# maxsonate/video-diffusion-nnx

Measured on AMD Instinct MI355X. Metric: denoised frames/sec, 16fx64x64 1000-step DDPM, higher is better.
Workload: dtype bf16; 1 GPU; config_v2_2 (north-star shape): Unet3D dim=64 C=1, 16f x 64x64, DDPM T=1000 p_sample_loop (UNet forward + p_sample per step, hipGraph replay); value = n_gpus*B*F/(T*s_per_step); batch_per_gpu=64, parallelism=dp1 (independent samples, no collective), mfma_operands=bf16, storage=weights fp32 master, activations bf16, fp32 accumulate, process_group=none (single process)

## Files before the change

### video_diffusion_nnx_amd/csrc/conv_igemm.hip

```cpp
#include "vdx_common.h"
#include <type_traits>
#include "vdx_internal.h"
#include "vdx_glds.h"
#include "model.h"
#include <stdlib.h>
#include <string.h>

namespace vdx {

typedef unsigned u32x4 __attribute__((ext_vector_type(4)));
typedef unsigned u32x2 __attribute__((ext_vector_type(2)));
constexpr unsigned OOB = 0xFFFFFFF0u;

template <int MODE, int BC, int TN, int NW, int INF>
__global__ __launch_bounds__(64 * NW, (NW == 8 && TN == 2) ? 4 : 2) void conv_igemm_kernel(const ConvArgs P) {
    using M = Mma<MODE>;
    constexpr int KT = M::KT;
    constexpr int RS = ROW_STRIDE;
    constexpr int WAVES_C = BC / 64;
    constexpr int WAVES_P = NW / WAVES_C;
    constexpr int NT = 64 * NW;
    constexpr int TM = 4;
    constexpr int APIECES = KT / 4;
    constexpr int WREGS = BC * 8 / NT;
// ... 732 lines not shown
    const int lp = lane & 15, q = lane >> 4;
    const int tiles_x = P.W >> 4, tiles_pf = tiles_x * (P.H >> 4);
    const int t0 = blockIdx.x * tiles_per_block, t1 = min(t0 + tiles_per_block, total_tiles);
    if (t0 >= t1) return;

    uint4 wf[9][2][2];
#pragma unroll
    for (int tap = 0; tap < 9; ++tap)
#pragma unroll
        for (int ch = 0; ch < 2; ++ch)
#pragma unroll
            for (int tm = 0; tm < 2; ++tm)
                wf[tap][ch][tm] = *reinterpret_cast<const uint4*>(reinterpret_cast<const char*>(P.wp) +
                    ((size_t)tap * P.wrows + P.wrow0 + wc * 32 + 8 * (lp >> 2) + 4 * tm + (lp & 3)) * 128 + ch * 64 + q * 16);
    if (tid < 128) chs[tid] = 0.0;
    if (tid < 64) biasl[tid] = P.bias ? P.bias[tid] : 0.f;

    const char* const zero_page = reinterpret_cast<const char*>(g_zero_page_c64d);
    const char* const xb = reinterpret_cast<const char*>(P.x0);
    const unsigned al_base = lds_addr(Al);
    auto decode = [&](int t, int& f, int& ty, int& tx) { f = t / tiles_pf; const int r = t - f * tiles_pf; ty = r / tiles_x; tx = r - ty * tiles_x; };
    auto dma = [&](int t, int buf) {
        int f, ty, tx; decode(t, f, ty, tx);
        int ln = lane;
        asm volatile("" : "+v"(ln));
        const unsigned dst = al_base + buf * C64D_APL + wave_u * 1024;
#pragma unroll
        for (int k = 0; k < NK; ++k) {
            if (wave_u + 8 * k >= NDMA) continue;
            const int hp = (wave_u + 8 * k) * 8 + (ln >> 3);
            const int hy = (hp * 3641) >> 16, hx = hp - hy * 18;
            const int gy = ty * 16 - 1 + hy, gx = tx * 16 - 1 + hx;
            const bool ok = hp < C64_HALO && gy >= 0 && gy < P.H && gx >= 0 && gx < P.W;
            const size_t off = (size_t)((f * P.H + gy) * P.W + gx) * 128 + (((ln & 7) ^ (hx & 7)) << 4);
            glds16(ok ? static_cast<const void*>(xb + off) : static_cast<const void*>(zero_page), dst + k * 8 * 1024);
        }
    };
    const __amdgpu_buffer_rsrc_t rsy = __builtin_amdgcn_make_buffer_rsrc(P.y, 0, (unsigned)P.NF * P.H * P.W * 64u * (OUT16 ? 2u : 4u), 0x00020000);
    f32x4 ssum[2], ssq[2];
#pragma unroll
    for (int i = 0; i < 2; ++i) { ssum[i] = f32x4{0.f, 0.f, 0.f, 0.f}; ssq[i] = f32x4{0.f, 0.f, 0.f, 0.f}; }
    auto flush_stats = [&](int b) {
        if (!P.out_stats) return;
#pragma unroll
        for (int tm = 0; tm < 2; ++tm)
#pragma unroll
            for (int e = 0; e < 4; ++e) {
                const float s1 = reduce16(ssum[tm][e]), s2 = reduce16(ssq[tm][e]);
                const int c = wc * 32 + 8 * q + 4 * tm + e;
                if (lp == 0) { unsafeAtomicAdd(&chs[c], (double)s1); unsafeAtomicAdd(&chs[64 + c], (double)s2); }
                ssum[tm][e] = 0.f; ssq[tm][e] = 0.f;
            }
        __syncthreads();
        const int cpg = 64 / P.out_groups;
        int tt = tid;
        asm volatile("" : "+v"(tt));
        if (tt < 2 * P.out_groups) {
            const int g = tt >> 1, which = tt & 1;
            double t = 0.0;
            for (int c = g * cpg; c < (g + 1) * cpg; ++c) t += chs[which * 64 + c];
            unsafeAtomicAdd(P.out_stats + (((size_t)b * GN_SLOTS + (blockIdx.x % GN_SLOTS)) * P.out_groups + g) * 2 + which, t);
        }
        __syncthreads();
        if (tid < 128) chs[tid] = 0.0;
        __syncthreads();
    };

    int bdx[3][2];
#pragma unroll
    for (int ch = 0; ch < 2; ++ch)
#pragma unroll
        for (int dx = 0; dx < 3; ++dx) { const int hx = lp + dx; bdx[dx][ch] = hx * 128 + 16 * ((q + 4 * ch) ^ (hx & 7)); }
    const int rowbase = (4 * wp) * 18 * 128;

    int fcur, tyc, txc;
    decode(t0, fcur, tyc, txc);
    int bcur = fcur / P.F;
    __syncthreads();
    dma(t0, 0);
    if (t0 + 1 < t1) { dma(t0 + 1, 1); wait_vm<5>(); } else wait_vm<0>();
    __syncthreads();
    int buf = 0;
    for (int t = t0; t < t1; ++t) {
        const bool more = t + 1 < t1, more2 = t + 2 < t1;
        int fn = fcur, tyn = tyc, txn = txc, bn = bcur;
        if (more) { decode(t + 1, fn, tyn, txn); bn = fn / P.F; }
        if (more2) dma(t + 2, buf >= 1 ? buf - 1 : 2);
        const char* At = Al + buf * C64D_APL + rowbase;
        const int oy0 = tyc * 16 + 4 * wp, ox = txc * 16 + lp;
        f32x4 acc[2][4];
        uint4 bf[2][3];
        auto frag_read = [&](uint4 (&d)[3], int hr, int ch) {
#pragma unroll
            for (int dx = 0; dx < 3; ++dx) d[dx] = *reinterpret_cast<const uint4*>(At + bdx[dx][ch] + hr * (18 * 128));
        };
        frag_read(bf[0], 0, 0);
#pragma unroll
        for (int hr = 0; hr < 6; ++hr) {
            if (hr < 4) { acc[0][hr] = f32x4{0.f, 0.f, 0.f, 0.f}; acc[1][hr] = f32x4{0.f, 0.f, 0.f, 0.f}; }
#pragma unroll
            for (int ch = 0; ch < 2; ++ch) {
                const int s_ = 2 * hr + ch;
                if (s_ + 1 < 12) frag_read(bf[(s_ + 1) & 1], (s_ + 1) >> 1, (s_ + 1) & 1);
                __builtin_amdgcn_sched_barrier(0);
#pragma unroll
                for (int dx = 0; dx < 3; ++dx)
#pragma unroll
                    for (int dy = 0; dy < 3; ++dy) {
                        const int tn = hr - dy;
                        if (tn < 0 || tn > 3) continue;
#pragma unroll
                        for (int tm = 0; tm < 2; ++tm) M::mma(acc[tm][tn], wf[dy * 3 + dx][ch][tm], bf[s_ & 1][dx]);
                    }
                __builtin_amdgcn_sched_barrier(0);
            }
            if (hr >= 2) {
                const int tn = hr - 2;
                float4 bias4[2];
#pragma unroll
                for (int tm = 0; tm < 2; ++tm) bias4[tm] = *reinterpret_cast<const float4*>(biasl + wc * 32 + 8 * q + 4 * tm);
                const unsigned gout = (unsigned)(((fcur * P.H + oy0 + tn) * P.W + ox) * 64 + wc * 32 + 8 * q);
                float4 v[2];
#pragma unroll
                for (int tm = 0; tm < 2; ++tm) {
                    v[tm] = make_float4(acc[tm][tn][0] + bias4[tm].x, acc[tm][tn][1] + bias4[tm].y, acc[tm][tn][2] + bias4[tm].z, acc[tm][tn][3] + bias4[tm].w);
                    ssum[tm][0] += v[tm].x; ssum[tm][1] += v[tm].y; ssum[tm][2] += v[tm].z; ssum[tm][3] += v[tm].w;
                    ssq[tm][0] += v[tm].x * v[tm].x; ssq[tm][1] += v[tm].y * v[tm].y; ssq[tm][2] += v[tm].z * v[tm].z; ssq[tm][3] += v[tm].w * v[tm].w;
                }
                if constexpr (OUT16)
                    __builtin_amdgcn_raw_buffer_store_b128(u32x4{pack_bf16x2(v[0].x, v[0].y), pack_bf16x2(v[0].z, v[0].w), pack_bf16x2(v[1].x, v[1].y), pack_bf16x2(v[1].z, v[1].w)}, rsy, gout * 2u, 0, 0);
                else {
#pragma unroll
                    for (int tm = 0; tm < 2; ++tm)
                        __builtin_amdgcn_raw_buffer_store_b128(u32x4{__float_as_uint(v[tm].x), __float_as_uint(v[tm].y), __float_as_uint(v[tm].z), __float_as_uint(v[tm].w)}, rsy, (gout + 4 * tm) * 4u, 0, 0);
                }
            }
        }
        constexpr int NST = OUT16 ? 4 : 8;
        if (more2) wait_vm<5 + NST>(); else wait_vm<NST>();
        if (more && bn != bcur) { flush_stats(bcur); bcur = bn; }
        fcur = fn; tyc = tyn; txc = txn;
        buf = buf == 2 ? 0 : buf + 1;
        __syncthreads();
    }
    flush_stats(bcur);
}

#ifndef VDX_C64Q_VPM
#define VDX_C64Q_VPM 6
#endif
template <int CIN, bool PRO, bool OUT16, int COUT = 64>
__global__ __launch_bounds__(512) void conv64q_kernel(const ConvArgs P, const int tiles_per_block, const int total_tiles) {
    using M = Mma<MODE_BF16>;
    static_assert(CIN == 64 || (CIN == 128 && !PRO), "prologue form: 64 input channels");
    static_assert(COUT == 64 || (COUT == 32 && !PRO), "COUT");
    constexpr int NWC = COUT / 16, NWP = 8 / NWC, RW = 16 / NWP, NHR = RW + 2, NSTEP = 2 * NHR;
    constexpr int NPL = CIN / 64;
    constexpr int NDMA = 41, NK = (NDMA + 7) / 8;
    constexpr int NST = (OUT16 ? 1 : 2) * (RW / 2);
    extern __shared__ __attribute__((aligned(16))) char smem[];
    char* Al = smem;
    double* chs = reinterpret_cast<double*>(Al + 3 * C64D_APL);
    float* biasl = reinterpret_cast<float*>(chs + 128);
    float* coefA = biasl + 64;
    float* coefD = coefA + 64;
    float* gmean = coefD + 64;

    const int tid = threadIdx.x, lane = tid & 63;
    const int wave_u = __builtin_amdgcn_readfirstlane(tid >> 6);
    const int wc = wave_u % NWC, wp = wave_u / NWC;
    const int lp = lane & 15, q = lane >> 4;
    const int tiles_x = P.W >> 4, tiles_pf = tiles_x * (P.H >> 4);
    const int t0 = blockIdx.x * tiles_per_block, t1 = min(t0 + tiles_per_block, total_tiles);
    if (t0 >= t1) return;

    uint4 wf[9][CIN / 32];
#pragma unroll
    for (int tap = 0; tap < 9; ++tap)
#pragma unroll
        for (int c = 0; c < CIN / 32; ++c)
            wf[tap][c] = *reinterpret_cast<const uint4*>(reinterpret_cast<const char*>(P.wp) +
                ((size_t)tap * P.wrows + P.wrow0 + wc * 16 + lp) * (CIN * 2) + c * 64 + q * 16);
    if (tid < 128) chs[tid] = 0.0;
    if (tid < 64) biasl[tid] = (P.bias && tid < COUT) ? P.bias[tid] : 0.f;

    const char* const zero_page = reinterpret_cast<const char*>(g_zero_page_c64d);
    const char* const xb0 = reinterpret_cast<const char*>(P.x0);
    const char* const xb1 = (CIN == 128) ? (P.C1 ? reinterpret_cast<const char*>(P.x1) : xb0 + 128) : xb0;
    const int rowb = (CIN == 128 && !P.C1) ? 256 : 128;
    const bool split32 = CIN == 64 && P.C1 == 32;
    const char* const xs1 = split32 ? reinterpret_cast<const char*>(P.x1) : nullptr;
    const unsigned al_base = lds_addr(Al);
    auto decode = [&](int t, int& f, int& ty, int& tx) { f = t / tiles_pf; const int r = t - f * tiles_pf; ty = r / tiles_x; tx = r - ty * tiles_x; };
    auto dma = [&](int t, int plane, int buf) {
        int f, ty, tx; decode(t, f, ty, tx);
        int ln = lane;
        asm volatile("" : "+v"(ln));
        const char* const xb = plane ? xb1 : xb0;
        const unsigned dst = al_base + buf * C64D_APL + wave_u * 1024;
#pragma unroll
        for (int k = 0; k < NK; ++k) {
            if (wave_u + 8 * k >= NDMA) continue;
            const int hp = (wave_u + 8 * k) * 8 + (ln >> 3);
            const int hy = (hp * 3641) >> 16, hx = hp - hy * 18;
            const int gy = ty * 16 - 1 + hy, gx = tx * 16 - 1 + hx;
            const bool ok = hp < C64_HALO && gy >= 0 && gy < P.H && gx >= 0 && gx < P.W;
            const int cch = (ln & 7) ^ (hx & 7);
            const size_t pixi = (size_t)((f * P.H + gy) * P.W + gx);
            const char* src = split32 ? (cch < 4 ? xb0 : xs1) + pixi * 64 + ((cch & 3) << 4) : xb + pixi * rowb + (cch << 4);
            glds16(ok ? static_cast<const void*>(src) : static_cast<const void*>(zero_page), dst + k * 8 * 1024);
        }
    };
    const __amdgpu_buffer_rsrc_t rsy = __builtin_amdgcn_make_buffer_rsrc(P.y, 0, (unsigned)P.NF * P.H * P.W * (unsigned)COUT * (OUT16 ? 2u : 4u), 0x00020000);
    float ssum[8], ssq[8];
#pragma unroll
    for (int i = 0; i < 8; ++i) { ssum[i] = 0.f; ssq[i] = 0.f; }
    auto flush_stats = [&](int b) {
        if (!P.out_stats) return;
#pragma unroll
        for (int i = 0; i < 8; ++i) {
            const float s1 = reduce16(ssum[i]), s2 = reduce16(ssq[i]);
            const int c = wc * 16 + 8 * (q >> 1) + i;
            if (lp == 0) { unsafeAtomicAdd(&chs[c], (double)s1); unsafeAtomicAdd(&chs[64 + c], (double)s2); }
            ssum[i] = 0.f; ssq[i] = 0.f;
        }
        __syncthreads();
        const int cpg = COUT / P.out_groups;
        int tt = tid;
        asm volatile("" : "+v"(tt));
        if (tt < 2 * P.out_groups) {
            const int g = tt >> 1, which = tt & 1;
            double t = 0.0;
            for (int c = g * cpg; c < (g + 1) * cpg; ++c) t += chs[which * 64 + c];
            unsafeAtomicAdd(P.out_stats + (((size_t)b * GN_SLOTS + (blockIdx.x % GN_SLOTS)) * P.out_groups + g) * 2 + which, t);
        }
        __syncthreads();
        if (tid < 128) chs[tid] = 0.0;
        __syncthreads();
    };
    const int tch = tid & 7, trow = tid >> 3;
    float ca[PRO ? 8 : 1], cd[PRO ? 8 : 1];
    auto make_coef = [&](int b) {
        if constexpr (PRO) {
            gn_mean_rstd_wg(P.in_stats, b, P.groups, (double)P.F * P.H * P.W * (64 / P.groups), gmean, tid, 512);
            __syncthreads();
            int tt = tid;
            asm volatile("" : "+v"(tt));
            if (tt < 64) {
                const int g = tt / (64 / P.groups);
                const float m = gmean[2 * g], rsd = gmean[2 * g + 1];
                float sc = 1.f, sh = 0.f;
                if (P.ss) { sc = P.ss[(size_t)b * P.ss_stride + tt] + 1.f; sh = P.ss[(size_t)b * P.ss_stride + 64 + tt]; }
                coefA[tt] = rsd * P.gamma[tt] * sc;
                coefD[tt] = (P.beta[tt] - m * rsd * P.gamma[tt]) * sc + sh;
            }
            __syncthreads();
#pragma unroll
            for (int i = 0; i < 8; ++i) { ca[i] = coefA[8 * tch + i]; cd[i] = coefD[8 * tch + i]; }
        }
    };
    auto piece_off = [&](int k) __attribute__((always_inline)) -> int {
        const int hp = trow + 64 * k;
        const int hy = (hp * 3641) >> 16, hx = hp - hy * 18;
        return hp * 128 + ((tch ^ (hx & 7)) << 4);
    };
    auto piece_ok = [&](int k, int ty, int tx) __attribute__((always_inline)) -> bool {
        const int hp = trow + 64 * k;
        const int hy = (hp * 3641) >> 16, hx = hp - hy * 18;
        const int gy = ty * 16 - 1 + hy, gx = tx * 16 - 1 + hx;
        return hp < C64_HALO && gy >= 0 && gy < P.H && gx >= 0 && gx < P.W;
    };
    auto piece_math = [&](u32x4 v, bool ok) __attribute__((always_inline)) -> u32x4 {
        const unsigned w4[4] = {v.x, v.y, v.z, v.w};
        unsigned o4[4];
#pragma unroll
        for (int j = 0; j < 4; ++j) {
            const float lo = silu_f(fmaf(__uint_as_float(w4[j] << 16), ca[PRO ? 2 * j : 0], cd[PRO ? 2 * j : 0]));
            const float hi = silu_f(fmaf(__uint_as_float(w4[j] & 0xFFFF0000u), ca[PRO ? 2 * j + 1 : 0], cd[PRO ? 2 * j + 1 : 0]));
            o4[j] = ok ? pack_bf16x2(lo, hi) : 0u;
        }
        return u32x4{o4[0], o4[1], o4[2], o4[3]};
    };
    constexpr int NPK = 6;
    auto piece_live = [&](int k) __attribute__((always_inline)) -> bool { return k < NPK - 1 || wave_u == 0; };

    int bdx[3][2];
#pragma unroll
    for (int ch = 0; ch < 2; ++ch)
#pragma unroll
        for (int dx = 0; dx < 3; ++dx) { const int hx = lp + dx; bdx[dx][ch] = hx * 128 + 16 * ((q + 4 * ch) ^ (hx & 7)); }
    const int rowbase = (RW * wp) * 18 * 128;

    int fcur, tyc, txc;
    decode(t0, fcur, tyc, txc);
    int bcur = fcur / P.F;
    __syncthreads();
    const int npass = (t1 - t0) * NPL;
    dma(t0, 0, 0);
    if (npass > 1) dma(NPL == 1 ? t0 + 1 : t0, NPL == 1 ? 0 : 1, 1);
    if (npass > 1 && !PRO) wait_vm<5>(); else wait_vm<0>();
    int bcoef = bcur;
    if constexpr (PRO) {
        make_coef(bcur);
#pragma unroll
        for (int k = 0; k < NPK; ++k) {
            if (!piece_live(k)) continue;
            char* pp = Al + piece_off(k);
            if (trow + 64 * k < C64D_AROWS) *reinterpret_cast<u32x4*>(pp) = piece_math(*reinterpret_cast<const u32x4*>(pp), piece_ok(k, tyc, txc));
        }
    }
    __syncthreads();
    int buf = 0, j = 0;
    f32x4 acc[RW];
    for (int t = t0; t < t1; ++t) {
        const bool more = t + 1 < t1;
        int fn = fcur, tyn = tyc, txn = txc, bn = bcur;
        if (more) { decode(t + 1, fn, tyn, txn); bn = fn / P.F; }
        const int oy0 = tyc * 16 + RW * wp, ox = txc * 16 + lp;
#pragma unroll
        for (int plane = 0; plane < NPL; ++plane, ++j) {
            if (j + 2 < npass) {
                const int j2 = j + 2;
                dma(t0 + j2 / NPL, NPL == 1 ? 0 : (j2 & 1), buf >= 1 ? buf - 1 : 2);
            }
            const int bufn = buf == 2 ? 0 : buf + 1;
            const char* At = Al + buf * C64D_APL + rowbase;
            char* const An = Al + bufn * C64D_APL;
            auto steps = [&](auto xf_tag) __attribute__((always_inline)) {
                constexpr bool XF = decltype(xf_tag)::value;
                uint4 bf[2][3];
                auto frag_read = [&](uint4 (&d)[3], int hr, int ch) __attribute__((always_inline)) {
#pragma unroll
                    for (int dx = 0; dx < 3; ++dx) d[dx] = *reinterpret_cast<const uint4*>(At + bdx[dx][ch] + hr * (18 * 128));
                };
                auto half_math = [&](unsigned w0, unsigned w1, int cb, bool ok, unsigned& o0, unsigned& o1) __attribute__((always_inline)) {
                    const float a0 = silu_f(fmaf(__uint_as_float(w0 << 16), ca[PRO ? cb : 0], cd[PRO ? cb : 0]));
                    const float a1 = silu_f(fmaf(__uint_as_float(w0 & 0xFFFF0000u), ca[PRO ? cb + 1 : 0], cd[PRO ? cb + 1 : 0]));
                    const float a2 = silu_f(fmaf(__uint_as_float(w1 << 16), ca[PRO ? cb + 2 : 0], cd[PRO ? cb + 2 : 0]));
                    const float a3 = silu_f(fmaf(__uint_as_float(w1 & 0xFFFF0000u), ca[PRO ? cb + 3 : 0], cd[PRO ? cb + 3 : 0]));
                    const unsigned keep = ok ? 0xFFFFFFFFu : 0u;
                    o0 = pack_bf16x2(a0, a1) & keep;
                    o1 = pack_bf16x2(a2, a3) & keep;
                };
                u32x4 pv = u32x4{0u, 0u, 0u, 0u}, cur = pv;
                bool pok = false, okc = false;
                unsigned oh0 = 0u, oh1 = 0u;
                if constexpr (XF) { pv = *reinterpret_cast<const u32x4*>(An + piece_off(0)); pok = piece_ok(0, tyn, txn); }
                frag_read(bf[0], 0, 0);
#pragma unroll
                for (int hr = 0; hr < NHR; ++hr) {
                    if (plane == 0 && hr < RW) acc[hr] = f32x4{0.f, 0.f, 0.f, 0.f};
#pragma unroll
                    for (int ch = 0; ch < 2; ++ch) {
                        const int s_ = 2 * hr + ch;
                        if (s_ + 1 < NSTEP) frag_read(bf[(s_ + 1) & 1], (s_ + 1) >> 1, (s_ + 1) & 1);
                        __builtin_amdgcn_sched_barrier(0);
#pragma unroll
                        for (int dx = 0; dx < 3; ++dx)
#pragma unroll
                            for (int dy = 0; dy < 3; ++dy) {
                                const int tn = hr - dy;
                                if (tn < 0 || tn > RW - 1) continue;
                                M::mma(acc[tn], wf[dy * 3 + dx][plane * 2 + ch], bf[s_ & 1][dx]);
                            }
                        if constexpr (XF) {
                            const int c = s_ - 4;
                            if (c >= 0 && c < 10) {
                                const int k = c >> 1;
                                if ((c & 1) == 0) {
                                    cur = pv; okc = pok;
                                    if (k + 1 < NPK - 1) { pv = *reinterpret_cast<const u32x4*>(An + piece_off(k + 1)); pok = piece_ok(k + 1, tyn, txn); }
                                    half_math(cur.x, cur.y, 0, okc, oh0, oh1);
                                } else {
                                    unsigned o2, o3;
                                    half_math(cur.z, cur.w, 4, okc, o2, o3);
                                    *reinterpret_cast<u32x4*>(An + piece_off(k)) = u32x4{oh0, oh1, o2, o3};
                                }
#pragma unroll
                                for (int i = 0; i < 9; ++i) { __builtin_amdgcn_sched_group_barrier(0x008, 1, 0); __builtin_amdgcn_sched_group_barrier(0x002, VDX_C64Q_VPM, 0); }
                            }
                        }
                        __builtin_amdgcn_sched_barrier(0);
                        if constexpr (XF) {
                            if (s_ == 14 && wave_u == 0 && trow + 64 * (NPK - 1) < C64D_AROWS) {
                                char* pp = An + piece_off(NPK - 1);
                                *reinterpret_cast<u32x4*>(pp) = piece_math(*reinterpret_cast<const u32x4*>(pp), piece_ok(NPK - 1, tyn, txn));
                            }
                        }
                    }
                    if (plane == NPL - 1 && hr >= 3 && (hr & 1)) {
                        const int ta = hr - 3;
                        float v[8];
#pragma unroll
                        for (int r = 0; r < 4; ++r) {
                            const auto sw = __builtin_amdgcn_permlane16_swap(__float_as_uint(acc[ta][r]), __float_as_uint(acc[ta + 1][r]), false, false);
                            v[r] = __uint_as_float(sw[0]); v[4 + r] = __uint_as_float(sw[1]);
                        }
                        const float4 b0 = *reinterpret_cast<const float4*>(biasl + wc * 16 + 8 * (q >> 1)), b1 = *reinterpret_cast<const float4*>(biasl + wc * 16 + 8 * (q >> 1) + 4);
                        v[0] += b0.x; v[1] += b0.y; v[2] += b0.z; v[3] += b0.w; v[4] += b1.x; v[5] += b1.y; v[6] += b1.z; v[7] += b1.w;
#pragma unroll
                        for (int i = 0; i < 8; ++i) { ssum[i] += v[i]; ssq[i] += v[i] * v[i]; }
                        const unsigned gout = (unsigned)(((fcur * P.H + oy0 + ta + (q & 1)) * P.W + ox) * COUT + wc * 16 + 8 * (q >> 1));
                        if constexpr (OUT16)
                            __builtin_amdgcn_raw_buffer_store_b128(u32x4{pack_bf16x2(v[0], v[1]), pack_bf16x2(v[2], v[3]), pack_bf16x2(v[4], v[5]), pack_bf16x2(v[6], v[7])}, rsy, gout * 2u, 0, 0);
                        else {
                            __builtin_amdgcn_raw_buffer_store_b128(u32x4{__float_as_uint(v[0]), __float_as_uint(v[1]), __float_as_uint(v[2]), __float_as_uint(v[3])}, rsy, gout * 4u, 0, 0);
                            __builtin_amdgcn_raw_buffer_store_b128(u32x4{__float_as_uint(v[4]), __float_as_uint(v[5]), __float_as_uint(v[6]), __float_as_uint(v[7])}, rsy, (gout + 4) * 4u, 0, 0);
                        }
                    }
                }
            };
            if (PRO && more) steps(std::true_type{}); else steps(std::false_type{});
            if constexpr (PRO) wait_vm<NST>();
            else {
                const bool issued = j + 2 < npass;
                if (plane == NPL - 1) { if (issued) wait_vm<5 + NST>(); else wait_vm<NST>(); }
                else { if (issued) wait_vm<5>(); else wait_vm<0>(); }
            }
            if (plane == NPL - 1) {
                if (more && bn != bcur) { flush_stats(bcur); bcur = bn; }
                if constexpr (PRO) {
                    if (t + 2 < t1) { int f2, ty2, tx2; decode(t + 2, f2, ty2, tx2); const int b2 = f2 / P.F; if (b2 != bcoef) { make_coef(b2); bcoef = b2; } }
                }
            }
            buf = bufn;
            __syncthreads();
        }
        fcur = fn; tyc = tyn; txc = txn;
    }
    flush_stats(bcur);
}

template <int MODE>
__global__ void pack_weights_kernel(const float* __restrict__ src, void* __restrict__ dst, int taps, int Cin, int Cout, int CinPad) {
    const size_t n = (size_t)taps * Cout * CinPad;
    for (size_t i = (size_t)blockIdx.x * blockDim.x + threadIdx.x; i < n; i += (size_t)gridDim.x * blockDim.x) {
        const int ci = (int)(i % CinPad);
        const size_t r = i / CinPad;
        const int co = (int)(r % Cout);
        const int t = (int)(r / Cout);
        const float v = (ci < Cin) ? src[((size_t)t * Cin + ci) * Cout + co] : 0.f;
        store_operand<MODE>(dst, i, v);
    }
}

template <int MODE>
__global__ void pack_weights_t_kernel(const float* __restrict__ src, void* __restrict__ dst, int taps, int Cin, int Cout, int CoutPad) {
    const size_t n = (size_t)taps * Cin * CoutPad;
    for (size_t i = (size_t)blockIdx.x * blockDim.x + threadIdx.x; i < n; i += (size_t)gridDim.x * blockDim.x) {
        const int co = (int)(i % CoutPad);
        const size_t r = i / CoutPad;
        const int ci = (int)(r % Cin);
        const int t = (int)(r / Cin);
        const float v = (co < Cout) ? src[((size_t)(taps - 1 - t) * Cin + ci) * Cout + co] : 0.f;
        store_operand<MODE>(dst, i, v);
    }
}

template <int MODE>
__global__ __launch_bounds__(256) void pack_jobs_kernel(const float* __restrict__ params, char* __restrict__ dst_base, const PackJob* __restrict__ jobs) {
    const PackJob J = jobs[blockIdx.y];
    const float* src = params + J.src;
    char* dstc = dst_base + J.dst;
    if (J.kind == 2) {
        for (int i = blockIdx.x * 256 + threadIdx.x; i < (int)J.n; i += gridDim.x * 256) reinterpret_cast<float*>(dstc)[i] = src[i];
        return;
    }
    if (J.kind == 0) {
        __shared__ float tile[32][33];
        const int tk = (J.Pad + 31) / 32, tc = (J.Cout + 31) / 32, per_tap = tk * tc, ntiles = J.taps * per_tap;
        const int tx = threadIdx.x & 31, ty = threadIdx.x >> 5;
        for (int id = blockIdx.x; id < ntiles; id += gridDim.x) {
            const int t = id / per_tap, rem = id - t * per_tap, kb = rem / tc, cb = rem - kb * tc;
#pragma unroll
            for (int j = 0; j < 4; ++j) {
                const int kk = kb * 32 + ty + 8 * j, co = cb * 32 + tx;
                tile[ty + 8 * j][tx] = (kk < J.Cin && co < J.Cout) ? src[((size_t)t * J.Cin + kk) * J.Cout + co] : 0.f;
            }
            __syncthreads();
#pragma unroll
            for (int j = 0; j < 4; ++j) {
                const int co = cb * 32 + ty + 8 * j, kk = kb * 32 + tx;
                if (co < J.Cout && kk < J.Pad) {
                    const size_t di = ((size_t)t * J.Cout + co) * J.Pad + kk;
                    const float v = tile[tx][ty + 8 * j];
                    store_operand<MODE>(dstc, di, v);
                }
            }
            __syncthreads();
        }
        return;
    }
    const int rows = (int)(J.n / J.Pad);
    for (int r = blockIdx.x; r < rows; r += gridDim.x) {
        const size_t drow = (size_t)r * J.Pad;
        if (false) {
        } else if (J.kind == 1) {
            const int t = r / J.Cin, ci = r - t * J.Cin;
            const float* srow = src + ((size_t)(J.taps - 1 - t) * J.Cin + ci) * J.Cout;
            for (int k = threadIdx.x; k < J.Pad; k += 256) {
                const float v = (k < J.Cout) ? srow[k] : 0.f;
                store_operand<MODE>(dstc, drow + k, v);
            }
        } else {
            for (int k = threadIdx.x; k < J.Pad; k += 256) {
                const int sel = k / J.Cout, kk = k - sel * J.Cout;
                const float* sp = params + (sel == 0 ? J.src : (sel == 1 ? J.src1 : J.src2));
                const float v = (sel < 3) ? sp[(size_t)r * J.Cout + kk] : 0.f;
                store_operand<MODE>(dstc, drow + k, v);
            }
        }
    }
}


static void choose_patch(int BM, int NF, int F, int Ho, int Wo, int stride, int K, int& PH, int& PW, int& NP) {
    int pw = 4;
    while (pw < Wo && pw < 16) pw *= 2;
    long best = -1;
    PH = BM / pw; PW = pw; NP = 1;
    for (int np = 1; np <= 16; np *= 2) {
        if (F % np) continue;
        const int ph = BM / (pw * np);
        if (ph < 1) continue;
        const int IH = (ph - 1) * stride + K, IW = (pw - 1) * stride + K;
        if ((long)np * IH * IW > 400) continue;
        const long blocks = (long)(NF / np) * ((Ho + ph - 1) / ph) * ((Wo + pw - 1) / pw);
        if (best < 0 || blocks < best) { best = blocks; PH = ph; PW = pw; NP = np; }
    }
}

size_t conv_packed_bytes(int mode, int taps, int Cin, int Cout) {
    const int KT = mode == MODE_F32 ? Mma<MODE_F32>::KT : Mma<MODE_BF16>::KT;
    const int ES = mode == MODE_F32 ? 4 : 2;
    const int CinPad = (Cin + KT - 1) / KT * KT;
    return (size_t)taps * Cout * CinPad * ES;
}

int conv_cin_pad(int mode, int Cin) {
    const int KT = mode == MODE_F32 ? Mma<MODE_F32>::KT : Mma<MODE_BF16>::KT;
    return (Cin + KT - 1) / KT * KT;
}

hipError_t launch_pack_weights(int mode, const float* src, void* dst, int taps, int Cin, int Cout, hipStream_t st) {
    const int CinPad = conv_cin_pad(mode, Cin);
    const size_t n = (size_t)taps * Cout * CinPad;
    const int blocks = (int)std::min<size_t>((n + 255) / 256, 2048);
    if (mode == MODE_F32) hipLaunchKernelGGL(pack_weights_kernel<MODE_F32>, dim3(blocks), dim3(256), 0, st, src, dst, taps, Cin, Cout, CinPad);
    else if (mode == MODE_F16) hipLaunchKernelGGL(pack_weights_kernel<MODE_F16>, dim3(blocks), dim3(256), 0, st, src, dst, taps, Cin, Cout, CinPad);
    else hipLaunchKernelGGL(pack_weights_kernel<MODE_BF16>, dim3(blocks), dim3(256), 0, st, src, dst, taps, Cin, Cout, CinPad);
    return hipGetLastError();
}

hipError_t launch_pack_jobs(int mode, const float* params, void* dst_base, const PackJob* d_jobs, int njobs, hipStream_t st) {
    if (njobs <= 0) return hipSuccess;
    dim3 grid(96, njobs);
    if (mode == MODE_F32) hipLaunchKernelGGL(pack_jobs_kernel<MODE_F32>, grid, dim3(256), 0, st, params, reinterpret_cast<char*>(dst_base), d_jobs);
    else if (mode == MODE_F16) hipLaunchKernelGGL(pack_jobs_kernel<MODE_F16>, grid, dim3(256), 0, st, params, reinterpret_cast<char*>(dst_base), d_jobs);
    else hipLaunchKernelGGL(pack_jobs_kernel<MODE_BF16>, grid, dim3(256), 0, st, params, reinterpret_cast<char*>(dst_base), d_jobs);
    return hipGetLastError();
}

hipError_t launch_pack_weights_t(int mode, const float* src, void* dst, int taps, int Cin, int Cout, hipStream_t st) {
    const int CoutPad = conv_cin_pad(mode, Cout);
    const size_t n = (size_t)taps * Cin * CoutPad;
    const int blocks = (int)std::min<size_t>((n + 255) / 256, 2048);
    if (mode == MODE_F32) hipLaunchKernelGGL(pack_weights_t_kernel<MODE_F32>, dim3(blocks), dim3(256), 0, st, src, dst, taps, Cin, Cout, CoutPad);
    else if (mode == MODE_F16) hipLaunchKernelGGL(pack_weights_t_kernel<MODE_F16>, dim3(blocks), dim3(256), 0, st, src, dst, taps, Cin, Cout, CoutPad);
    else hipLaunchKernelGGL(pack_weights_t_kernel<MODE_BF16>, dim3(blocks), dim3(256), 0, st, src, dst, taps, Cin, Cout, CoutPad);
    return hipGetLastError();
}

static ConvWork conv_work(int mode, const ConvArgs& a) {
    ConvWork w;
    const double es = mode == MODE_F32 ? 4.0 : 2.0;
    const int taps = a.kind ? 16 : a.kh * a.kw;
    const double ho = a.kind ? 2.0 * a.H : (a.H + a.stride - 1) / a.stride, wo = a.kind ? 2.0 * a.W : (a.W + a.stride - 1) / a.stride;
    const double cin = a.C0 + a.C1;
    w.flops = 2.0 * a.NF * ho * wo * cin * a.Cout * (a.kind ? 4 : taps);
    w.bytes = (double)a.NF * a.H * a.W * (a.C0 * (a.x0_bf16 ? 2.0 : 4.0) + a.C1 * (a.x1_bf16 ? 2.0 : 4.0)) + a.NF * ho * wo * a.Cout * (a.y_bf16 ? 2.0 : 4.0)
            + (a.res ? a.NF * ho * wo * a.Cout * (a.res_bf16 ? 2.0 : 4.0) : 0.0) + es * taps * cin * a.Cout;
    snprintf(w.shape, sizeof(w.shape), "%s%dx%d %d->%d %dx%dx%d%s%s%s%s", a.kind ? "convT" : "conv", a.kind ? 4 : a.kh, a.kind ? 4 : a.kw, a.C0 + a.C1, a.Cout,
             a.NF, a.H, a.W, a.stride == 2 ? " s2" : "", a.pro ? " +prologue" : "", a.res ? " +res" : "", a.C1 ? " concat" : "");
// ... 155 lines not shown
```

Measured before the change: 49.16 frames/s.

## Register-prefetch halo tiles two ahead in prologue conv64q, double-buffer LDS

Moves the GroupNorm+SiLU prologue variant of conv64q into its own specialised function. Halo pieces for tile t+2 are loaded with buffer loads straight into registers, then normalised and written into the other LDS buffer while the MMAs for the current tile run. This replaces the old path that used a triple-buffered LDS DMA and did read-modify-write of raw data in LDS. The aim is to cut LDS round trips and hide global latency; the cost is higher register pressure (12 u32x4 held across the loop), which could lower occupancy or cause spills.

```diff
diff --git a/video_diffusion_nnx_amd/csrc/conv_igemm.hip b/video_diffusion_nnx_amd/csrc/conv_igemm.hip
--- a/video_diffusion_nnx_amd/csrc/conv_igemm.hip
+++ b/video_diffusion_nnx_amd/csrc/conv_igemm.hip
@@ -908,8 +908,9 @@
 template <int CIN, bool PRO, bool OUT16, int COUT = 64>
 __global__ __launch_bounds__(512) void conv64q_kernel(const ConvArgs P, const int tiles_per_block, const int total_tiles) {
     using M = Mma<MODE_BF16>;
-    static_assert(CIN == 64 || (CIN == 128 && !PRO), "prologue form: 64 input channels");
-    static_assert(COUT == 64 || (COUT == 32 && !PRO), "COUT");
+    static_assert(!PRO, "the prologue form is the specialisation below");
+    static_assert(CIN == 64 || CIN == 128, "CIN");
+    static_assert(COUT == 64 || COUT == 32, "COUT");
     constexpr int NWC = COUT / 16, NWP = 8 / NWC, RW = 16 / NWP, NHR = RW + 2, NSTEP = 2 * NHR;
     constexpr int NPL = CIN / 64;
     constexpr int NDMA = 41, NK = (NDMA + 7) / 8;
@@ -918,9 +919,6 @@
     char* Al = smem;
     double* chs = reinterpret_cast<double*>(Al + 3 * C64D_APL);
     float* biasl = reinterpret_cast<float*>(chs + 128);
-    float* coefA = biasl + 64;
-    float* coefD = coefA + 64;
-    float* gmean = coefD + 64;
 
     const int tid = threadIdx.x, lane = tid & 63;
     const int wave_u = __builtin_amdgcn_readfirstlane(tid >> 6);
@@ -994,52 +992,6 @@
         if (tid < 128) chs[tid] = 0.0;
         __syncthreads();
     };
-    const int tch = tid & 7, trow = tid >> 3;
-    float ca[PRO ? 8 : 1], cd[PRO ? 8 : 1];
-    auto make_coef = [&](int b) {
-        if constexpr (PRO) {
-            gn_mean_rstd_wg(P.in_stats, b, P.groups, (double)P.F * P.H * P.W * (64 / P.groups), gmean, tid, 512);
-            __syncthreads();
-            int tt = tid;
-            asm volatile("" : "+v"(tt));
-            if (tt < 64) {
-                const int g = tt / (64 / P.groups);
-                const float m = gmean[2 * g], rsd = gmean[2 * g + 1];
-                float sc = 1.f, sh = 0.f;
-                if (P.ss) { sc = P.ss[(size_t)b * P.ss_stride + tt] + 1.f; sh = P.ss[(size_t)b * P.ss_stride + 64 + tt]; }
-                coefA[tt] = rsd * P.gamma[tt] * sc;
-                coefD[tt] = (P.beta[tt] - m * rsd * P.gamma[tt]) * sc + sh;
-            }
-            __syncthreads();
-#pragma unroll
-            for (int i = 0; i < 8; ++i) { ca[i] = coefA[8 * tch + i]; cd[i] = coefD[8 * tch + i]; }
-        }
-    };
-    auto piece_off = [&](int k) __attribute__((always_inline)) -> int {
-        const int hp = trow + 64 * k;
-        const int hy = (hp * 3641) >> 16, hx = hp - hy * 18;
-        return hp * 128 + ((tch ^ (hx & 7)) << 4);
-    };
-    auto piece_ok = [&](int k, int ty, int tx) __attribute__((always_inline)) -> bool {
-        const int hp = trow + 64 * k;
-        const int hy = (hp * 3641) >> 16, hx = hp - hy * 18;
-        const int gy = ty * 16 - 1 + hy, gx = tx * 16 - 1 + hx;
-        return hp < C64_HALO && gy >= 0 && gy < P.H && gx >= 0 && gx < P.W;
-    };
-    auto piece_math = [&](u32x4 v, bool ok) __attribute__((always_inline)) -> u32x4 {
-        const unsigned w4[4] = {v.x, v.y, v.z, v.w};
-        unsigned o4[4];
-#pragma unroll
-        for (int j = 0; j < 4; ++j) {
-            const float lo = silu_f(fmaf(__uint_as_float(w4[j] << 16), ca[PRO ? 2 * j : 0], cd[PRO ? 2 * j : 0]));
-            const float hi = silu_f(fmaf(__uint_as_float(w4[j] & 0xFFFF0000u), ca[PRO ? 2 * j + 1 : 0], cd[PRO ? 2 * j + 1 : 0]));
-            o4[j] = ok ? pack_bf16x2(lo, hi) : 0u;
-        }
-        return u32x4{o4[0], o4[1], o4[2], o4[3]};
-    };
-    constexpr int NPK = 6;
-    auto piece_live = [&](int k) __attribute__((always_inline)) -> bool { return k < NPK - 1 || wave_u == 0; };
-
     int bdx[3][2];
 #pragma unroll
     for (int ch = 0; ch < 2; ++ch)
@@ -1054,17 +1006,7 @@
     const int npass = (t1 - t0) * NPL;
     dma(t0, 0, 0);
     if (npass > 1) dma(NPL == 1 ? t0 + 1 : t0, NPL == 1 ? 0 : 1, 1);
-    if (npass > 1 && !PRO) wait_vm<5>(); else wait_vm<0>();
-    int bcoef = bcur;
-    if constexpr (PRO) {
-        make_coef(bcur);
-#pragma unroll
-        for (int k = 0; k < NPK; ++k) {
-            if (!piece_live(k)) continue;
-            char* pp = Al + piece_off(k);
-            if (trow + 64 * k < C64D_AROWS) *reinterpret_cast<u32x4*>(pp) = piece_math(*reinterpret_cast<const u32x4*>(pp), piece_ok(k, tyc, txc));
-        }
-    }
+    if (npass > 1) wait_vm<5>(); else wait_vm<0>();
     __syncthreads();
     int buf = 0, j = 0;
     f32x4 acc[RW];
@@ -1081,27 +1023,12 @@
             }
             const int bufn = buf == 2 ? 0 : buf + 1;
             const char* At = Al + buf * C64D_APL + rowbase;
-            char* const An = Al + bufn * C64D_APL;
-            auto steps = [&](auto xf_tag) __attribute__((always_inline)) {
-                constexpr bool XF = decltype(xf_tag)::value;
+            auto steps = [&]() __attribute__((always_inline)) {
                 uint4 bf[2][3];
                 auto frag_read = [&](uint4 (&d)[3], int hr, int ch) __attribute__((always_inline)) {
 #pragma unroll
                     for (int dx = 0; dx < 3; ++dx) d[dx] = *reinterpret_cast<const uint4*>(At + bdx[dx][ch] + hr * (18 * 128));
                 };
-                auto half_math = [&](unsigned w0, unsigned w1, int cb, bool ok, unsigned& o0, unsigned& o1) __attribute__((always_inline)) {
-                    const float a0 = silu_f(fmaf(__uint_as_float(w0 << 16), ca[PRO ? cb : 0], cd[PRO ? cb : 0]));
-                    const float a1 = silu_f(fmaf(__uint_as_float(w0 & 0xFFFF0000u), ca[PRO ? cb + 1 : 0], cd[PRO ? cb + 1 : 0]));
-                    const float a2 = silu_f(fmaf(__uint_as_float(w1 << 16), ca[PRO ? cb + 2 : 0], cd[PRO ? cb + 2 : 0]));
-                    const float a3 = silu_f(fmaf(__uint_as_float(w1 & 0xFFFF0000u), ca[PRO ? cb + 3 : 0], cd[PRO ? cb + 3 : 0]));
-                    const unsigned keep = ok ? 0xFFFFFFFFu : 0u;
-                    o0 = pack_bf16x2(a0, a1) & keep;
-                    o1 = pack_bf16x2(a2, a3) & keep;
-                };
-                u32x4 pv = u32x4{0u, 0u, 0u, 0u}, cur = pv;
-                bool pok = false, okc = false;
-                unsigned oh0 = 0u, oh1 = 0u;
-                if constexpr (XF) { pv = *reinterpret_cast<const u32x4*>(An + piece_off(0)); pok = piece_ok(0, tyn, txn); }
                 frag_read(bf[0], 0, 0);
 #pragma unroll
                 for (int hr = 0; hr < NHR; ++hr) {
@@ -1119,30 +1046,7 @@
                                 if (tn < 0 || tn > RW - 1) continue;
                                 M::mma(acc[tn], wf[dy * 3 + dx][plane * 2 + ch], bf[s_ & 1][dx]);
                             }
-                        if constexpr (XF) {
-                            const int c = s_ - 4;
-                            if (c >= 0 && c < 10) {
-                                const int k = c >> 1;
-                                if ((c & 1) == 0) {
-                                    cur = pv; okc = pok;
-                                    if (k + 1 < NPK - 1) { pv = *reinterpret_cast<const u32x4*>(An + piece_off(k + 1)); pok = piece_ok(k + 1, tyn, txn); }
-                                    half_math(cur.x, cur.y, 0, okc, oh0, oh1);
-                                } else {
-                                    unsigned o2, o3;
-                                    half_math(cur.z, cur.w, 4, okc, o2, o3);
-                                    *reinterpret_cast<u32x4*>(An + piece_off(k)) = u32x4{oh0, oh1, o2, o3};
-                                }
-#pragma unroll
-                                for (int i = 0; i < 9; ++i) { __builtin_amdgcn_sched_group_barrier(0x008, 1, 0); __builtin_amdgcn_sched_group_barrier(0x002, VDX_C64Q_VPM, 0); }
-                            }
-                        }
                         __builtin_amdgcn_sched_barrier(0);
-                        if constexpr (XF) {
-                            if (s_ == 14 && wave_u == 0 && trow + 64 * (NPK - 1) < C64D_AROWS) {
-                                char* pp = An + piece_off(NPK - 1);
-                                *reinterpret_cast<u32x4*>(pp) = piece_math(*reinterpret_cast<const u32x4*>(pp), piece_ok(NPK - 1, tyn, txn));
-                            }
-                        }
                     }
                     if (plane == NPL - 1 && hr >= 3 && (hr & 1)) {
                         const int ta = hr - 3;
@@ -1166,18 +1070,14 @@
                     }
                 }
             };
-            if (PRO && more) steps(std::true_type{}); else steps(std::false_type{});
-            if constexpr (PRO) wait_vm<NST>();
-            else {
+            steps();
+            {
                 const bool issued = j + 2 < npass;
                 if (plane == NPL - 1) { if (issued) wait_vm<5 + NST>(); else wait_vm<NST>(); }
                 else { if (issued) wait_vm<5>(); else wait_vm<0>(); }
             }
             if (plane == NPL - 1) {
                 if (more && bn != bcur) { flush_stats(bcur); bcur = bn; }
-                if constexpr (PRO) {
-                    if (t + 2 < t1) { int f2, ty2, tx2; decode(t + 2, f2, ty2, tx2); const int b2 = f2 / P.F; if (b2 != bcoef) { make_coef(b2); bcoef = b2; } }
-                }
             }
             buf = bufn;
             __syncthreads();
@@ -1185,6 +1085,251 @@
         fcur = fn; tyc = tyn; txc = txn;
     }
     flush_stats(bcur);
+}
+
+template <bool OUT16>
+__device__ __forceinline__ void conv64q_pro_tiles(const ConvArgs& P, const int tiles_per_block, const int total_tiles) {
+    using M = Mma<MODE_BF16>;
+    constexpr int NWC = 4, NWP = 2, RW = 8, NHR = RW + 2, NSTEP = 2 * NHR;
+    constexpr int NPK = 6;
+    extern __shared__ __attribute__((aligned(16))) char smem[];
+    char* Al = smem;
+    double* chs = reinterpret_cast<double*>(Al + 3 * C64D_APL);
+    float* biasl = reinterpret_cast<float*>(chs + 128);
+    float* coefA = biasl + 64;
+    float* coefD = coefA + 64;
+    float* gmean = coefD + 64;
+
+    const int tid = threadIdx.x, lane = tid & 63;
+    const int wave_u = __builtin_amdgcn_readfirstlane(tid >> 6);
+    const int wc = wave_u % NWC, wp = wave_u / NWC;
+    const int lp = lane & 15, q = lane >> 4;
+    const int tiles_x = P.W >> 4, tiles_pf = tiles_x * (P.H >> 4);
+    const int t0 = blockIdx.x * tiles_per_block, t1 = min(t0 + tiles_per_block, total_tiles);
+    if (t0 >= t1) return;
+
+    uint4 wf[9][2];
+#pragma unroll
+    for (int tap = 0; tap < 9; ++tap)
+#pragma unroll
+        for (int c = 0; c < 2; ++c)
+            wf[tap][c] = *reinterpret_cast<const uint4*>(reinterpret_cast<const char*>(P.wp) +
+                ((size_t)tap * P.wrows + P.wrow0 + wc * 16 + lp) * 128 + c * 64 + q * 16);
+    if (tid < 128) chs[tid] = 0.0;
+    if (tid < 64) biasl[tid] = P.bias ? P.bias[tid] : 0.f;
+
+    auto decode = [&](int t, int& f, int& ty, int& tx) { f = t / tiles_pf; const int r = t - f * tiles_pf; ty = r / tiles_x; tx = r - ty * tiles_x; };
+    const __amdgpu_buffer_rsrc_t rsy = __builtin_amdgcn_make_buffer_rsrc(P.y, 0, (unsigned)P.NF * P.H * P.W * 64u * (OUT16 ? 2u : 4u), 0x00020000);
+    const unsigned xbytes = (unsigned)P.NF * P.H * P.W * 128u;
+    const __amdgpu_buffer_rsrc_t rsx = __builtin_amdgcn_make_buffer_rsrc(const_cast<float*>(P.x0), 0, xbytes, 0x00020000);
+    float ssum[8], ssq[8];
+#pragma unroll
+    for (int i = 0; i < 8; ++i) { ssum[i] = 0.f; ssq[i] = 0.f; }
+    auto flush_stats = [&](int b) {
+        if (!P.out_stats) return;
+#pragma unroll
+        for (int i = 0; i < 8; ++i) {
+            const float s1 = reduce16(ssum[i]), s2 = reduce16(ssq[i]);
+            const int c = wc * 16 + 8 * (q >> 1) + i;
+            if (lp == 0) { unsafeAtomicAdd(&chs[c], (double)s1); unsafeAtomicAdd(&chs[64 + c], (double)s2); }
+            ssum[i] = 0.f; ssq[i] = 0.f;
+        }
+        __syncthreads();
+        const int cpg = 64 / P.out_groups;
+        int tt = tid;
+        asm volatile("" : "+v"(tt));
+        if (tt < 2 * P.out_groups) {
+            const int g = tt >> 1, which = tt & 1;
+            double t = 0.0;
+            for (int c = g * cpg; c < (g + 1) * cpg; ++c) t += chs[which * 64 + c];
+            unsafeAtomicAdd(P.out_stats + (((size_t)b * GN_SLOTS + (blockIdx.x % GN_SLOTS)) * P.out_groups + g) * 2 + which, t);
+        }
+        __syncthreads();
+        if (tid < 128) chs[tid] = 0.0;
+        __syncthreads();
+    };
+    const int tch = tid & 7, trow = tid >> 3;
+    float ca[8], cd[8];
+    auto make_coef = [&](int b) {
+        gn_mean_rstd_wg(P.in_stats, b, P.groups, (double)P.F * P.H * P.W * (64 / P.groups), gmean, tid, 512);
+        __syncthreads();
+        int tt = tid;
+        asm volatile("" : "+v"(tt));
+        if (tt < 64) {
+            const int g = tt / (64 / P.groups);
+            const float m = gmean[2 * g], rsd = gmean[2 * g + 1];
+            float sc = 1.f, sh = 0.f;
+            if (P.ss) { sc = P.ss[(size_t)b * P.ss_stride + tt] + 1.f; sh = P.ss[(size_t)b * P.ss_stride + 64 + tt]; }
+            coefA[tt] = rsd * P.gamma[tt] * sc;
+            coefD[tt] = (P.beta[tt] - m * rsd * P.gamma[tt]) * sc + sh;
+        }
+        __syncthreads();
+#pragma unroll
+        for (int i = 0; i < 8; ++i) { ca[i] = coefA[8 * tch + i]; cd[i] = coefD[8 * tch + i]; }
+    };
+    int pyx[NPK];
+#pragma unroll
+    for (int k = 0; k < NPK; ++k) {
+        const int hp = trow + 64 * k;
+        const int hy = (hp * 3641) >> 16, hx = hp - hy * 18;
+        pyx[k] = ((hp < C64_HALO ? hy : (1 << 20)) << 5) | hx;
+    }
+    auto piece_pos = [&](int k) __attribute__((always_inline)) -> int { int p = pyx[k]; asm volatile("" : "+v"(p)); return p; };
+    auto piece_off = [&](int k, int p) __attribute__((always_inline)) -> int { return (trow + 64 * k) * 128 + ((tch ^ (p & 7)) << 4); };
+    auto piece_math = [&](u32x4 v, bool ok) __attribute__((always_inline)) -> u32x4 {
+        const unsigned w4[4] = {v.x, v.y, v.z, v.w};
+        unsigned o4[4];
+#pragma unroll
+        for (int j = 0; j < 4; ++j) {
+            const float lo = silu_f(fmaf(__uint_as_float(w4[j] << 16), ca[2 * j], cd[2 * j]));
+            const float hi = silu_f(fmaf(__uint_as_float(w4[j] & 0xFFFF0000u), ca[2 * j + 1], cd[2 * j + 1]));
+            o4[j] = ok ? pack_bf16x2(lo, hi) : 0u;
+        }
+        return u32x4{o4[0], o4[1], o4[2], o4[3]};
+    };
+    u32x4 rs[2][NPK];
+    unsigned okm[2] = {0u, 0u};
+    auto fetch = [&](int t, auto set_tag) __attribute__((always_inline)) {
+        constexpr int S = decltype(set_tag)::value;
+        int f, ty, tx; decode(t, f, ty, tx);
+        const int y0 = ty * 16 - 1, x0 = tx * 16 - 1, row0 = f * P.H;
+        const bool live = t < t1;
+        unsigned off[NPK], m = 0u;
+#pragma unroll
+        for (int k = 0; k < NPK; ++k) {
+            const int p = piece_pos(k);
+            const int gy = y0 + (p >> 5), gx = x0 + (p & 31);
+            const bool ok = live & ((unsigned)gy < (unsigned)P.H) & ((unsigned)gx < (unsigned)P.W);
+            off[k] = ok ? (unsigned)((row0 + gy) * P.W + gx) * 128u + (unsigned)(tch << 4) : xbytes;
+            m |= (ok ? 1u : 0u) << k;
+        }
+        okm[S] = m;
+#pragma unroll
+        for (int k = 0; k < NPK; ++k) rs[S][k] = __builtin_amdgcn_raw_buffer_load_b128(rsx, off[k], 0, 0);
+    };
+    auto piece_ok = [&](int k, unsigned m) __attribute__((always_inline)) -> bool { return (m >> k) & 1u; };
+    int bdx[3][2];
+#pragma unroll
+    for (int ch = 0; ch < 2; ++ch)
+#pragma unroll
+        for (int dx = 0; dx < 3; ++dx) { const int hx = lp + dx; bdx[dx][ch] = hx * 128 + 16 * ((q + 4 * ch) ^ (hx & 7)); }
+    const int rowbase = (RW * wp) * 18 * 128;
+
+    int fcur, tyc, txc;
+    decode(t0, fcur, tyc, txc);
+    int bcur = fcur / P.F, bcoef = bcur;
+    __syncthreads();
+    fetch(t0, std::integral_constant<int, 0>{});
+    fetch(t0 + 1, std::integral_constant<int, 1>{});
+    make_coef(bcur);
+#pragma unroll
+    for (int k = 0; k < NPK; ++k)
+        if ((k < NPK - 1 || wave_u == 0) && trow + 64 * k < C64D_AROWS) *reinterpret_cast<u32x4*>(Al + piece_off(k, piece_pos(k))) = piece_math(rs[0][k], piece_ok(k, okm[0]));
+    asm volatile("" :: "v"(rs[0][NPK - 1]));
+    if (t0 + 1 < t1) { int f1, ty1, tx1; decode(t0 + 1, f1, ty1, tx1); const int b1 = f1 / P.F; if (b1 != bcoef) { make_coef(b1); bcoef = b1; } }
+    __syncthreads();
+
+    f32x4 acc[RW];
+    auto tile_pass = [&](const int t, auto par_tag) __attribute__((always_inline)) {
+        constexpr int PAR = decltype(par_tag)::value;
+        int fn = fcur, tyn = tyc, txn = txc, bn = bcur;
+        if (t + 1 < t1) { decode(t + 1, fn, tyn, txn); bn = fn / P.F; }
+        const int oy0 = tyc * 16 + RW * wp, ox = txc * 16 + lp;
+        fetch(t + 2, par_tag);
+        const char* At = Al + PAR * C64D_APL + rowbase;
+        char* const An = Al + (1 - PAR) * C64D_APL;
+        const u32x4 (&rn)[NPK] = rs[1 - PAR];
+        uint4 bf[2][3];
+        auto frag_read = [&](uint4 (&d)[3], int hr, int ch) __attribute__((always_inline)) {
+#pragma unroll
+            for (int dx = 0; dx < 3; ++dx) d[dx] = *reinterpret_cast<const uint4*>(At + bdx[dx][ch] + hr * (18 * 128));
+        };
+        auto half_math = [&](unsigned w0, unsigned w1, int cb, bool ok, unsigned& o0, unsigned& o1) __attribute__((always_inline)) {
+            const float a0 = silu_f(fmaf(__uint_as_float(w0 << 16), ca[cb], cd[cb]));
+            const float a1 = silu_f(fmaf(__uint_as_float(w0 & 0xFFFF0000u), ca[cb + 1], cd[cb + 1]));
+            const float a2 = silu_f(fmaf(__uint_as_float(w1 << 16), ca[cb + 2], cd[cb + 2]));
+            const float a3 = silu_f(fmaf(__uint_as_float(w1 & 0xFFFF0000u), ca[cb + 3], cd[cb + 3]));
+            const unsigned keep = ok ? 0xFFFFFFFFu : 0u;
+            o0 = pack_bf16x2(a0, a1) & keep;
+            o1 = pack_bf16x2(a2, a3) & keep;
+        };
+        bool okc = false;
+        unsigned oh0 = 0u, oh1 = 0u;
+        frag_read(bf[0], 0, 0);
+#pragma unroll
+        for (int hr = 0; hr < NHR; ++hr) {
+            if (hr < RW) acc[hr] = f32x4{0.f, 0.f, 0.f, 0.f};
+#pragma unroll
+            for (int ch = 0; ch < 2; ++ch) {
+                const int s_ = 2 * hr + ch;
+                if (s_ + 1 < NSTEP) frag_read(bf[(s_ + 1) & 1], (s_ + 1) >> 1, (s_ + 1) & 1);
+                __builtin_amdgcn_sched_barrier(0);
+#pragma unroll
+                for (int dx = 0; dx < 3; ++dx)
+#pragma unroll
+                    for (int dy = 0; dy < 3; ++dy) {
+                        const int tn = hr - dy;
+                        if (tn < 0 || tn > RW - 1) continue;
+                        M::mma(acc[tn], wf[dy * 3 + dx][ch], bf[s_ & 1][dx]);
+                    }
+                const int c = s_ - 4;
+                if (c >= 0 && c < 10) {
+                    const int k = c >> 1;
+                    if ((c & 1) == 0) {
+                        okc = piece_ok(k, okm[1 - PAR]);
+                        half_math(rn[k].x, rn[k].y, 0, okc, oh0, oh1);
+                    } else {
+                        unsigned o2, o3;
+                        half_math(rn[k].z, rn[k].w, 4, okc, o2, o3);
+                        *reinterpret_cast<u32x4*>(An + piece_off(k, piece_pos(k))) = u32x4{oh0, oh1, o2, o3};
+                    }
+#pragma unroll
+                    for (int i = 0; i < 9; ++i) { __builtin_amdgcn_sched_group_barrier(0x008, 1, 0); __builtin_amdgcn_sched_group_barrier(0x002, VDX_C64Q_VPM, 0); }
+                }
+                __builtin_amdgcn_sched_barrier(0);
+                if (s_ == 14 && wave_u == 0 && trow + 64 * (NPK - 1) < C64D_AROWS)
+                    *reinterpret_cast<u32x4*>(An + piece_off(NPK - 1, piece_pos(NPK - 1))) = piece_math(rn[NPK - 1], piece_ok(NPK - 1, okm[1 - PAR]));
+                if (s_ == 14) asm volatile("" :: "v"(rn[NPK - 1]));
+            }
+            if (hr >= 3 && (hr & 1)) {
+                const int ta = hr - 3;
+                float v[8];
+#pragma unroll
+                for (int r = 0; r < 4; ++r) {
+                    const auto sw = __builtin_amdgcn_permlane16_swap(__float_as_uint(acc[ta][r]), __float_as_uint(acc[ta + 1][r]), false, false);
+                    v[r] = __uint_as_float(sw[0]); v[4 + r] = __uint_as_float(sw[1]);
+                }
+                const float4 b0 = *reinterpret_cast<const float4*>(biasl + wc * 16 + 8 * (q >> 1)), b1 = *reinterpret_cast<const float4*>(biasl + wc * 16 + 8 * (q >> 1) + 4);
+                v[0] += b0.x; v[1] += b0.y; v[2] += b0.z; v[3] += b0.w; v[4] += b1.x; v[5] += b1.y; v[6] += b1.z; v[7] += b1.w;
+#pragma unroll
+                for (int i = 0; i < 8; ++i) { ssum[i] += v[i]; ssq[i] += v[i] * v[i]; }
+                const unsigned gout = (unsigned)(((fcur * P.H + oy0 + ta + (q & 1)) * P.W + ox) * 64 + wc * 16 + 8 * (q >> 1));
+                if constexpr (OUT16)
+                    __builtin_amdgcn_raw_buffer_store_b128(u32x4{pack_bf16x2(v[0], v[1]), pack_bf16x2(v[2], v[3]), pack_bf16x2(v[4], v[5]), pack_bf16x2(v[6], v[7])}, rsy, gout * 2u, 0, 0);
+                else {
+                    __builtin_amdgcn_raw_buffer_store_b128(u32x4{__float_as_uint(v[0]), __float_as_uint(v[1]), __float_as_uint(v[2]), __float_as_uint(v[3])}, rsy, gout * 4u, 0, 0);
+                    __builtin_amdgcn_raw_buffer_store_b128(u32x4{__float_as_uint(v[4]), __float_as_uint(v[5]), __float_as_uint(v[6]), __float_as_uint(v[7])}, rsy, (gout + 4) * 4u, 0, 0);
+                }
+            }
+        }
+        if (t + 1 < t1 && bn != bcur) { flush_stats(bcur); bcur = bn; }
+        if (t + 2 < t1) { int f2, ty2, tx2; decode(t + 2, f2, ty2, tx2); const int b2 = f2 / P.F; if (b2 != bcoef) { make_coef(b2); bcoef = b2; } }
+        __syncthreads();
+        fcur = fn; tyc = tyn; txc = txn;
+    };
+    for (int t = t0;;) {
+        tile_pass(t, std::integral_constant<int, 0>{});
+        if (++t >= t1) break;
+        tile_pass(t, std::integral_constant<int, 1>{});
+        if (++t >= t1) break;
+    }
+    flush_stats(bcur);
+}
+template <> __global__ __launch_bounds__(512) void conv64q_kernel<64, true, true, 64>(const ConvArgs P, const int tiles_per_block, const int total_tiles) {
+    conv64q_pro_tiles<true>(P, tiles_per_block, total_tiles);
+}
+template <> __global__ __launch_bounds__(512) void conv64q_kernel<64, true, false, 64>(const ConvArgs P, const int tiles_per_block, const int total_tiles) {
+    conv64q_pro_tiles<false>(P, tiles_per_block, total_tiles);
 }
 
 template <int MODE>
```

After: 49.44 frames/s, median of 6. About the same (+0.6%).
